# dackey-wav/3d-reconstruction-tool

Measured on AMD Instinct MI355X. Metric: Mpixel-hypotheses/s (PatchMatch sweep), higher is better.
Workload: dtype f32; 1 GPU; BASELINE config 3: 16-view 1920x1080 PatchMatch MVS, 8 iters x (2+8) hypotheses, 7x7 NCC, 4 sources, fast arithmetic; views_per_gpu=16, scene_views=16, width=1920, height=1080, patch=7, iters=8, samples=8, arithmetic=fast, sampling=u8-pairs, tile_rows=18, views_per_launch=4, schedule=auto, exchange=depth + normal + confidence maps once per sweep

## Files before the change

3d-reconstruction-tool_amd/_lib.py:

```python
import ctypes as C
import os

_HERE = os.path.dirname(os.path.abspath(__file__))
LIB_PATH = os.environ.get("AMVS_LIB") or os.path.join(_HERE, "libamvs.so")

AMVS_MAX_SRC = 6
MODES = {"default": 0, "exact": 1, "fast": 2}
SCHEDULES = {"auto": 0, "view-major": 1, "band-major": 2, "split": 3, "paired": 4}
SUPPORTED_PATCH_SIZES = tuple(range(3, 32, 2))
TSDF_MAX_POINTS = 1 << 27

f32p = C.POINTER(C.c_float)
i32p = C.POINTER(C.c_int)


class PmParams(C.Structure):
    _fields_ = [("patch_size", C.c_int32), ("num_iterations", C.c_int32),
                ("num_samples", C.c_int32), ("tile_rows", C.c_int32), ("views_per_launch", C.c_int32),
                ("depth_min", C.c_float), ("depth_max", C.c_float),
                ("log_depth_scale", C.c_float), ("log_depth_min", C.c_float), ("mode", C.c_int32),
                ("schedule", C.c_int32), ("first_iteration", C.c_int32), ("flags", C.c_int32)]


PM_NO_CONFIDENCE = 1
# ... 2 lines not shown
class XpmParams(C.Structure):
    _fields_ = [("patch_size", C.c_int32), ("window_stride", C.c_int32), ("num_refine", C.c_int32),
                ("view_propagation", C.c_int32), ("depth_min", C.c_float), ("depth_max", C.c_float),
                ("log_depth_scale", C.c_float), ("log_depth_min", C.c_float),
                ("consistency_px", C.c_float), ("consistency_rel", C.c_float)]


class Timing(C.Structure):
    _fields_ = [("init_ms", C.c_double), ("sweep_ms", C.c_double), ("confidence_ms", C.c_double),
                ("sweep_launches", C.c_int64), ("pixel_hypotheses", C.c_int64)]


SIGNATURES = {
    "amvs_version": (C.c_char_p, []),
    "amvs_last_error": (C.c_char_p, [C.c_void_p]),
    "amvs_create": (C.c_int, [C.c_int, C.c_int, C.c_int, C.c_int, f32p, f32p, C.POINTER(C.c_void_p)]),
    "amvs_destroy": (C.c_int, [C.c_void_p]),
    "amvs_set_stream": (C.c_int, [C.c_void_p, C.c_void_p]),
    "amvs_sync": (C.c_int, [C.c_void_p]),
    "amvs_set_view": (C.c_int, [C.c_void_p, C.c_int, f32p, f32p, f32p]),
    "amvs_set_view_device": (C.c_int, [C.c_void_p, C.c_int, C.c_void_p, f32p, f32p]),
    "amvs_set_view_bgr8": (C.c_int, [C.c_void_p, C.c_int, C.POINTER(C.c_uint8), C.c_int, C.c_int, f32p, f32p,
                                     C.POINTER(C.c_uint8)]),
    "amvs_patchmatch": (C.c_int, [C.c_void_p, C.c_int, i32p, i32p, C.c_int, C.POINTER(PmParams),
                                  C.c_uint64, f32p, f32p, f32p]),
    "amvs_patchmatch_device": (C.c_int, [C.c_void_p, C.c_int, i32p, i32p, C.c_int,
                                         C.POINTER(PmParams), C.c_uint64,
                                         C.c_void_p, C.c_void_p, C.c_void_p]),
    "amvs_get_timing": (C.c_int, [C.c_void_p, C.POINTER(Timing)]),
    "amvs_sampling_mode": (C.c_int, [C.c_void_p]),
    "amvs_set_sampling": (C.c_int, [C.c_void_p, C.c_int]),
    "amvs_set_mode": (C.c_int, [C.c_void_p, C.c_int]),
    "amvs_get_mode": (C.c_int, [C.c_void_p]),
    "amvs_set_sweep_tuning": (C.c_int, [C.c_void_p, C.c_int, C.c_int]),
    "amvs_set_split_tuning": (C.c_int, [C.c_void_p, C.c_int, C.c_int, C.c_int]),
    "amvs_set_step_tuning": (C.c_int, [C.c_void_p, C.c_int, i32p, i32p]),
    "amvs_set_step_timing": (C.c_int, [C.c_void_p, C.c_int]),
    "amvs_get_step_times": (C.c_int, [C.c_void_p, f32p, C.c_int, i32p]),
    "amvs_last_tile_rows": (C.c_int, [C.c_void_p]),
    "amvs_last_views_per_launch": (C.c_int, [C.c_void_p]),
    "amvs_plane_sweep": (C.c_int, [C.c_void_p, C.c_int, i32p, C.c_int, f32p, C.c_int, C.c_int,
                                   C.c_float, f32p, f32p]),
    "amvs_plane_sweep_device": (C.c_int, [C.c_void_p, C.c_int, i32p, i32p, C.c_int, f32p, C.c_int,
                                          C.c_int, C.c_float, C.c_void_p, C.c_void_p]),
    "amvs_plane_sweep_batch": (C.c_int, [C.c_void_p, C.c_int, i32p, i32p, C.c_int, f32p, C.c_int, C.c_int, C.c_float]),
    "amvs_fetch_sweep_maps": (C.c_int, [C.c_void_p, C.c_int, C.c_int, f32p, f32p]),
# ... 100 lines not shown
```

3d-reconstruction-tool_amd/core/dense_stereo.py:

```python
import threading
import time
from typing import Dict, List, Optional, Tuple

import numpy as np

from .camera import Camera, CameraPose
from .imageprep import prepare_views
from .. import engine as _engine
from .. import parallel as _parallel


def _torch_cuda():
    try:
        import torch
    except Exception:
        return None
    return torch if torch.cuda.is_available() else None


_DRAW_BUF = threading.local()


class DenseStereoReconstructor:
    NUM_NEIGHBORS = 6
# ... 4 lines not shown
                 process_group=None, device_prep: Optional[bool] = None):
        self.camera = camera
        self.scale = scale
        self.num_depths = num_depths
        self.patch_size = patch_size
        self.min_views = min_views
        self.consistency_thresh = consistency_thresh
        self.device_id = _parallel.local_device() if device is None else int(device)
        self.device_filter = device_filter
        self.process_group = process_group
        from . import imageprep as _ip
        self.device_prep = (_ip._cv is None) if device_prep is None else bool(device_prep)
        if mode not in ("exact", "fast"):
            raise ValueError("mode must be 'exact' or 'fast'")
        self.mode = mode
        print(f"Dense stereo using GPU: HIP device {self.device_id} (gfx950 kernels)")
        self.K_scaled = camera.K.copy()
        for r, c in ((0, 0), (1, 1), (0, 2), (1, 2)):
            self.K_scaled[r, c] *= scale
        self._engine = None
        self._engine_key = None
        self._engine_images = None
        self._resident_colors = False
        self._slot = {}

    def reconstruct(self, images: List[dict], poses: Dict[int, CameraPose],
                    max_pairs: int = 30) -> Tuple[np.ndarray, np.ndarray]:
        print("\n" + "=" * 60)
        print("GPU DENSE STEREO")
        print(f"  Scale: {self.scale}x, Depths: {self.num_depths}, Min views: {self.min_views}")
        print("=" * 60)
        t0 = time.time()
        camera_indices = sorted(poses.keys())
        n_cameras = len(camera_indices)
        if n_cameras < 3:
            print("Need at least 3 cameras for multi-view stereo")
            return np.array([]), np.array([])

        print("\nPreparing images...")
        if self.device_prep:
            processed = self._prepare_images_device(images, camera_indices, poses)
        else:
            processed = self._prepare_images(images, camera_indices)

        centers = np.array([poses[idx].center for idx in camera_indices])
        radius = np.percentile(np.linalg.norm(centers - np.median(centers, axis=0), axis=1), 90)
# ... 130 lines not shown

    def _draw_without_replacement(self, total: int, size: int) -> np.ndarray:
        buf = getattr(_DRAW_BUF, "pair", None)
        if buf is None or buf[0].size < total:
            cap = max(int(total), 1 << 20)
            buf = _DRAW_BUF.pair = (np.arange(cap, dtype=np.int64), np.empty(cap, np.int64))
        idx = buf[1][:total]
        np.copyto(idx, buf[0][:total])
        np.random.shuffle(idx)
        return idx[:size]

    def _prepare_images(self, images: List[dict], indices: List[int]) -> Dict:
        return dict(zip(indices, prepare_views([images[idx]["image"] for idx in indices], self.scale)))

    def _prepare_images_device(self, images: List[dict], indices: List[int], poses: Dict[int, CameraPose]) -> Dict:
        h, w = images[indices[0]]["image"].shape[:2]
        H, W = int(h * self.scale), int(w * self.scale)
        eng = self._engine
        if eng is None or not eng.reusable_for(H, W, len(indices), self.K_scaled, self.device_id, self.mode):
            if eng is not None:
                eng.close()
                self._engine = None
            eng = _engine.Engine(H, W, len(indices), self.K_scaled.astype(np.float32), device=self.device_id, mode=self.mode)
        self._slot = {idx: s for s, idx in enumerate(indices)}
        prepared = {}
        for idx in indices:
            img = images[idx]["image"]
            same = (H, W) == tuple(img.shape[:2])
            color = eng.set_view_bgr8(self._slot[idx], img, poses[idx].R, poses[idx].t, want_color=not same)
            prepared[idx] = {"color": img if same else color, "gray": None, "shape": (H, W)}
        self._engine, self._engine_images, self._resident_colors = eng, prepared, True
        self._engine_key = self._make_engine_key(prepared, poses)
        return prepared

    def _make_engine_key(self, processed: Dict, poses: Dict[int, CameraPose]):
        indices = sorted(processed.keys())
        H, W = processed[indices[0]]["shape"]
        pose_print = b"".join(np.asarray(poses[i].R, np.float64).tobytes() + np.asarray(poses[i].t, np.float64).tobytes()
                              for i in indices)
        return (tuple(indices), (int(H), int(W)), pose_print, self.K_scaled.tobytes(), self.device_id)

    def _find_neighbors(self, ref_idx: int, all_indices: List[int],
                        poses: Dict[int, CameraPose], k: int = 6) -> List[int]:
        c_ref = poses[ref_idx].center
        ranked = sorted(((idx, np.linalg.norm(poses[idx].center - c_ref))
                         for idx in all_indices if idx != ref_idx), key=lambda item: item[1])
        return [idx for idx, _ in ranked[:k]]

    def _ensure_engine(self, processed: Dict, poses: Dict[int, CameraPose]):
        indices = sorted(processed.keys())
        H, W = processed[indices[0]]["shape"]
        key = self._make_engine_key(processed, poses)
        if self._engine is not None and self._engine_images is processed and self._engine_key == key:
            return self._engine
# ... 79 lines not shown
```

3d-reconstruction-tool_amd/core/mvs_patchmatch.py:

```python
import time
from dataclasses import dataclass
from typing import Dict, List, Optional, Tuple

import numpy as np

from .camera import Camera, CameraPose
from .imageprep import prepare_view, prepare_views
from .. import engine as _engine
from .. import parallel as _parallel


@dataclass
class DepthNormalMap:
    depth: np.ndarray
    normal: np.ndarray
    confidence: np.ndarray


@dataclass
class _ResidentMaps:
    ref_ids: list
    depth: object
    normal: object
    confidence: object
# ... 34 lines not shown
        self.num_iterations = num_iterations
        self.num_samples = num_samples
        self.min_views = min_views
        self.depth_min = depth_min
        self.depth_max = depth_max
        self.seed = seed
        self.views_per_batch = max(1, int(views_per_batch))
        self.process_group = process_group
        self.device_fusion = device_fusion
        self.device_prep = (not _imageprep_has_cv2()) if device_prep is None else bool(device_prep)
        self.gather_normals = gather_normals
        self.extended = extended
        if mode not in ("exact", "fast"):
            raise ValueError("mode must be 'exact' or 'fast'")
        self.mode = mode
        self.device_id = _parallel.local_device() if device is None else int(device)
        print(f"PatchMatch MVS using GPU: HIP device {self.device_id} (gfx950 kernels)")
        self.K_scaled = camera.K.copy()
        self.K_scaled[:2] *= scale
        self._engine = None
        self._engine_key = None
        self._engine_images = None
        self._resident_colors = False
        self._slot = {}
        self.last_timing = None

    def reconstruct(self, images: List[dict], poses: Dict[int, CameraPose],
                    sparse_points: np.ndarray = None) -> Tuple[np.ndarray, np.ndarray]:
        points, colors, _ = self._reconstruct_maps(images, poses, sparse_points)
        return points, colors

    def reconstruct_mesh(self, images: List[dict], poses: Dict[int, CameraPose], sparse_points: np.ndarray = None, *,
                         voxel_size: Optional[float] = None, bounds=None, trunc_voxels: float = 4.0,
                         max_dim: int = 256) -> Tuple[np.ndarray, np.ndarray, np.ndarray]:
        rank, world = _parallel.rank_world(self.process_group)
        if world > 1:
            raise NotImplementedError("reconstruct_mesh runs on one process: meshing with a process group of "
                                      f"{world} ranks is not implemented (call it without a process group)")
        if trunc_voxels <= 0:
            raise ValueError("trunc_voxels must be positive")
        points, _, maps = self._reconstruct_maps(images, poses, sparse_points)
        empty = (np.zeros((0, 3), np.float32), np.zeros((0, 3), np.int32), np.zeros((0, 3), np.uint8))
        if maps is None or (bounds is None and len(points) == 0):
            return empty
        origin, voxel, dims, trunc = self._mesh_grid(points, bounds, voxel_size, trunc_voxels, max_dim)
        print(f"\nMeshing: {dims[0]} x {dims[1]} x {dims[2]} TSDF grid, voxel {voxel:.4g}, truncation {trunc:.4g}")
# ... 128 lines not shown
                    pooled.extend(z)
            if pooled:
                self.depth_min = max(0.1, np.percentile(pooled, 1))
                self.depth_max = np.percentile(pooled, 99) * 1.5
                return
        spread = np.linalg.norm(centers - np.median(centers, axis=0), axis=1)
        scene_scale = np.percentile(spread, 90)
        self.depth_min = max(0.1, scene_scale * 0.05)
        self.depth_max = scene_scale * 10.0

    def _prepare_images(self, images: List[dict], indices: List[int]) -> Dict:
        prepared = prepare_views([images[idx]["image"] for idx in indices], self.scale)
        return dict(zip(indices, prepared))

    def _prepare_images_device(self, images: List[dict], indices: List[int], poses: Dict[int, CameraPose]) -> Dict:
        h, w = images[indices[0]]["image"].shape[:2]
        H, W = int(h * self.scale), int(w * self.scale)
        eng = self._engine
        if eng is None or not eng.reusable_for(H, W, len(indices), self.K_scaled, self.device_id):
            if eng is not None:
                eng.close()
                self._engine = None
            eng = _engine.Engine(H, W, len(indices), self.K_scaled.astype(np.float32), device=self.device_id)
        self._slot = {idx: s for s, idx in enumerate(indices)}
        prepared = {}
        for idx in indices:
            img = images[idx]["image"]
            if img.shape[:2] != (h, w):
                raise ValueError("all views must share one size")
            same = (H, W) == (h, w)
            color = eng.set_view_bgr8(self._slot[idx], img, poses[idx].R, poses[idx].t, want_color=not same)
            prepared[idx] = {"color": img if same else color, "gray": None, "shape": (H, W)}
        self._engine, self._engine_images, self._resident_colors = eng, prepared, True
        self._engine_key = self._make_engine_key(prepared, poses, indices)
        return prepared

    def _make_engine_key(self, images: Dict, poses: Dict[int, CameraPose], indices: List[int]):
        H, W = images[indices[0]]["shape"]
        pose_print = b"".join(np.asarray(poses[i].R, np.float64).tobytes() + np.asarray(poses[i].t, np.float64).tobytes()
                              for i in indices)
        return (tuple(indices), (int(H), int(W)), pose_print, self.K_scaled.tobytes(), self.device_id)

    def _select_source_views(self, ref_idx: int, all_indices: List[int],
                             poses: Dict[int, CameraPose], k: int = 4) -> List[int]:
        c_ref = poses[ref_idx].center
        z_ref = poses[ref_idx].R[2, :]
        scored = []
        for idx in all_indices:
            if idx == ref_idx:
                continue
            baseline = np.linalg.norm(poses[idx].center - c_ref)
            cosang = np.clip(np.dot(z_ref, poses[idx].R[2, :]), -1, 1)
            angle = np.degrees(np.arccos(cosang))
            score = baseline * (1 - abs(angle - 20) / 60) if 5 < angle < 60 else 0
            scored.append((idx, score))
        scored.sort(key=lambda item: item[1], reverse=True)
# ... 339 lines not shown
```

3d-reconstruction-tool_amd/csrc/amvs_capi.hip:

```cpp
#include "../../include/amvs.h"
#include "amvs_kernels.h"
#include "amvs_buffer.h"

#include <dlfcn.h>
#include <rccl/rccl.h>

#include <array>
#include <cmath>
#include <cstdio>
#include <cstdlib>
#include <cstring>
#include <map>
#include <memory>
#include <string>
#include <vector>

static_assert(AMVS_MAX_SRC == AMVS_KMAX_SRC, "source-count limits out of sync");

#ifdef AMVS_CHECK_INDICES
namespace amvs {
void check_fetch_kernels(unsigned long long out[4], bool reset);
void check_fetch_kernels_fast(unsigned long long out[4], bool reset);
void check_fetch_sweep_fast(unsigned long long out[4], bool reset);
void check_fetch_sweep_exact(unsigned long long out[4], bool reset);
void check_fetch_generic(unsigned long long out[4], bool reset);
void check_fetch_extended(unsigned long long out[4], bool reset);
void check_fetch_fusion(unsigned long long out[4], bool reset);
void check_fetch_knn(unsigned long long out[4], bool reset);
void check_fetch_mesh(unsigned long long out[4], bool reset);
}
#endif

namespace {

std::string g_create_error;

void index_report(uint64_t out[4], bool reset)
{
    out[0] = out[1] = out[2] = out[3] = 0;
#ifdef AMVS_CHECK_INDICES
    (void)hipDeviceSynchronize();
    void (*const fetch[])(unsigned long long[4], bool) = {
        amvs::check_fetch_kernels, amvs::check_fetch_kernels_fast, amvs::check_fetch_sweep_fast, amvs::check_fetch_sweep_exact,
        amvs::check_fetch_generic, amvs::check_fetch_extended, amvs::check_fetch_fusion, amvs::check_fetch_knn,
        amvs::check_fetch_mesh};
    for (auto f : fetch) {
        unsigned long long r[4] = {0, 0, 0, 0};
        f(r, reset);
        if (r[0] && !out[0]) { out[1] = r[1]; out[2] = r[2]; out[3] = r[3]; }
        out[0] += r[0];
    }
#else
    (void)reset;
#endif
}

struct Stats {
    amvs::DeviceBuffer<float> mean, var;
    std::vector<char> done;
};

struct FastStats {
    amvs::DeviceBuffer<float2> maps;
    std::vector<char> done;
};

struct Cloud {
    amvs::DeviceBuffer<double> pts;
    amvs::DeviceBuffer<unsigned char> rgb;
    long long n = 0;
};

}

struct amvs_ctx {
    int device = 0, H = 0, W = 0, n_views = 0, n_cu = 256;
    long long stride = 0;
    float K[9], Kinv[9];
    std::vector<std::array<float, 9>> R;
    std::vector<std::array<float, 3>> t;
    std::vector<char> have;
    amvs::ScratchCache cache;
    amvs::DeviceBuffer<float> d_images;
    amvs::DeviceBuffer<uint16_t> d_pairs;
    long long pstride = 0;
    amvs::DeviceBuffer<unsigned char> d_bgr;
    amvs::DeviceBuffer<unsigned char> d_prep_src;
    amvs::DeviceBuffer<int> d_prep_tab;
    std::vector<char> have_bgr;
    amvs::DeviceBuffer<int> d_flag;
    mutable std::vector<char> exact8;
    mutable bool flags_dirty = false;
    bool force_f32 = false;
    int mode = AMVS_MODE_EXACT;
    int default_band_major = 0;
    int sweep_tile_rows = 0, sweep_chunk = 0;
    int sweep_key8 = 1;
    std::map<int, Stats> stats;
    std::map<int, FastStats> fstats;
    amvs::DeviceBuffer<float> d_depth[2], d_cost, d_normal[2], d_aux;
    amvs::DeviceBuffer<amvs::Job> d_jobs;
    amvs::DeviceBuffer<float> d_planes;
    amvs::DeviceBuffer<unsigned> d_keys;
    amvs::DeviceBuffer<float> d_xcand_d, d_xcand_n;
    amvs::DeviceBuffer<int> d_xsrc;
    amvs::DeviceBuffer<float> d_sweep_depth, d_sweep_conf;
    int n_sweep = 0;
    Cloud cloud;
    std::unique_ptr<amvs::TsdfState, void (*)(amvs::TsdfState *)> tsdf{nullptr, amvs::tsdf_state_free};
    amvs::DeviceBuffer<float> d_samples;
    std::vector<hipStream_t> split_streams;
// ... 647 lines not shown
    c->stream = c->own_stream;
    for (auto &ev : c->ev) HIPCHK(nullptr, hipEventCreate(&ev));
    HIPCHK(nullptr, c->d_images.reserve(c->stride * n_views, c->cache));
    HIPCHK(nullptr, hipMemsetAsync(c->d_images.get(), 0, sizeof(float) * c->stride * n_views, c->stream));
    HIPCHK(nullptr, c->d_pairs.reserve(c->pstride * n_views, c->cache));
    HIPCHK(nullptr, hipMemsetAsync(c->d_pairs.get(), 0, sizeof(uint16_t) * c->pstride * n_views, c->stream));
    HIPCHK(nullptr, c->d_flag.reserve(n_views, c->cache));
    HIPCHK(nullptr, hipMemsetAsync(c->d_flag.get(), 0, sizeof(int) * n_views, c->stream));
    *out = c.release();
    return AMVS_OK;
}

int amvs_destroy(amvs_ctx *c)
{
    if (!c) return AMVS_OK;
    (void)hipSetDevice(c->device);
    if (c->stream) (void)hipStreamSynchronize(c->stream);
    (void)amvs_comm_destroy(c);
    for (auto &st : c->split_streams) (void)hipStreamDestroy(st);
    for (auto &ev : c->split_events) (void)hipEventDestroy(ev);
    for (auto &ev : c->ev) if (ev) (void)hipEventDestroy(ev);
    for (auto &ev : c->ev_groups) (void)hipEventDestroy(ev);
    for (auto &ev : c->ev_steps) (void)hipEventDestroy(ev);
    if (c->own_stream) (void)hipStreamDestroy(c->own_stream);
    delete c;
    return AMVS_OK;
}

int amvs_set_stream(amvs_ctx *c, void *hip_stream)
{
    if (!c) return AMVS_EINVAL;
    c->stream = hip_stream ? (hipStream_t)hip_stream : c->own_stream;
    return AMVS_OK;
}

int amvs_sync(amvs_ctx *c)
{
    if (!c) return AMVS_EINVAL;
    int rc = bind_device(c);
    if (rc) return rc;
    HIPCHK(c, hipStreamSynchronize(c->stream));
    resolve_timing(c);
    return checked(c, AMVS_OK);
}

static int view_uploaded(amvs_ctx *c, int view, const float R[9], const float t[3], bool sync)
// ... 25 lines not shown
    if ((rc = view_uploaded(c, view, R, t, kind == hipMemcpyHostToDevice))) return rc;
    return checked(c, AMVS_OK);
}

static void resize_axis_tables(int n_dst, int n_src, std::vector<int> &ofs, std::vector<short> &w, bool clamp_ofs)
{
    const double scale = 1.0 / ((double)n_dst / (double)n_src);
    ofs.resize(n_dst); w.resize(2 * (size_t)n_dst);
    for (int d = 0; d < n_dst; ++d) {
        float f = (float)((d + 0.5) * scale - 0.5);
        int s = (int)std::floor(f);
        f -= (float)s;
        if (clamp_ofs) {
            if (s < 0) { f = 0.f; s = 0; }
            if (s >= n_src - 1) { f = 0.f; s = n_src - 1; }
        }
        ofs[d] = s;
        const float c0 = 1.f - f, c1 = f;
        w[2 * d] = (short)std::nearbyint(c0 * 2048.f);
        w[2 * d + 1] = (short)std::nearbyint(c1 * 2048.f);
    }
}

int amvs_set_view_bgr8(amvs_ctx *c, int view, const uint8_t *bgr_host, int src_h, int src_w, const float R[9],
                       const float t[3], uint8_t *scaled_bgr_out)
{
    if (c) c->pm_resumable = false;
    if (!c) return AMVS_EINVAL;
    if (view < 0 || view >= c->n_views || !bgr_host || !R || !t || src_h < 1 || src_w < 1)
        return fail(c, AMVS_EINVAL, "bad view argument");
    int rc = bind_device(c);
    if (rc) return rc;
    const size_t n_src = (size_t)src_h * src_w, n_dst = (size_t)c->H * c->W;
    std::vector<int> xofs, yofs;
    std::vector<short> ialpha, ibeta;
    resize_axis_tables(c->W, src_w, xofs, ialpha, true);
    resize_axis_tables(c->H, src_h, yofs, ibeta, false);
    HIPCHK(c, c->d_bgr.reserve(3 * n_dst * (size_t)c->n_views, c->cache));
    unsigned char *d_scaled = c->d_bgr.get() + 3 * n_dst * (size_t)view;
    const size_t tab_ints = (size_t)c->W + c->H, tab_shorts = 2 * ((size_t)c->W + c->H);
    HIPCHK(c, c->d_prep_src.reserve(3 * n_src, c->cache));
    HIPCHK(c, c->d_prep_tab.reserve(tab_ints + tab_shorts / 2, c->cache));
    unsigned char *d_src = c->d_prep_src.get();
    int *d_xofs = c->d_prep_tab.get(), *d_yofs = d_xofs + c->W;
    short *d_ialpha = (short *)(d_xofs + tab_ints), *d_ibeta = d_ialpha + 2 * c->W;
    HIPCHK(c, hipMemcpyAsync(d_src, bgr_host, 3 * n_src, hipMemcpyHostToDevice, c->stream));
    HIPCHK(c, hipMemcpyAsync(d_xofs, xofs.data(), 4 * (size_t)c->W, hipMemcpyHostToDevice, c->stream));
    HIPCHK(c, hipMemcpyAsync(d_yofs, yofs.data(), 4 * (size_t)c->H, hipMemcpyHostToDevice, c->stream));
    HIPCHK(c, hipMemcpyAsync(d_ialpha, ialpha.data(), 4 * (size_t)c->W, hipMemcpyHostToDevice, c->stream));
    HIPCHK(c, hipMemcpyAsync(d_ibeta, ibeta.data(), 4 * (size_t)c->H, hipMemcpyHostToDevice, c->stream));
    HIPCHK(c, amvs::launch_prep_bgr8(d_src, src_h, src_w, c->H, c->W, d_xofs, d_ialpha, d_yofs, d_ibeta, d_scaled,
                                     c->d_images.get() + view * c->stride, c->stream));
    if (scaled_bgr_out) HIPCHK(c, hipMemcpyAsync(scaled_bgr_out, d_scaled, 3 * n_dst, hipMemcpyDeviceToHost, c->stream));
    if ((rc = view_uploaded(c, view, R, t, true))) return rc;
    c->have_bgr[view] = 1;
    return checked(c, AMVS_OK);
}

int amvs_set_view_colors(amvs_ctx *c, int view, const uint8_t *bgr_host)
{
    if (!c) return AMVS_EINVAL;
    if (view < 0 || view >= c->n_views || !bgr_host) return fail(c, AMVS_EINVAL, "bad view argument");
    int rc = bind_device(c);
    if (rc) return rc;
    const size_t n = (size_t)c->H * c->W;
    HIPCHK(c, c->d_bgr.reserve(3 * n * (size_t)c->n_views, c->cache));
    HIPCHK(c, hipMemcpyAsync(c->d_bgr.get() + 3 * n * (size_t)view, bgr_host, 3 * n, hipMemcpyHostToDevice, c->stream));
    HIPCHK(c, hipStreamSynchronize(c->stream));
    c->have_bgr[view] = 1;
    return checked(c, AMVS_OK);
}

int amvs_set_view(amvs_ctx *c, int view, const float *gray_host, const float R[9], const float t[3])
{
    return set_view_common(c, view, gray_host, R, t, hipMemcpyHostToDevice);
}

int amvs_set_view_device(amvs_ctx *c, int view, const void *gray_device, const float R[9], const float t[3])
{
// ... 1038 lines not shown
```

3d-reconstruction-tool_amd/csrc/amvs_prep.hip:

```cpp
#include "amvs_kernels.h"

namespace amvs {

__global__ __launch_bounds__(256) void prep_resize_bgr8_kernel(const unsigned char *__restrict__ src, int sh, int sw,
                                                               int dh, int dw, const int *__restrict__ xofs,
                                                               const short *__restrict__ ialpha,
                                                               const int *__restrict__ yofs,
                                                               const short *__restrict__ ibeta,
                                                               unsigned char *__restrict__ dst)
{
    const long long n = (long long)dh * dw;
    for (long long i = (long long)blockIdx.x * blockDim.x + threadIdx.x; i < n;
         i += (long long)gridDim.x * blockDim.x) {
        const int dy = (int)(i / dw), dx = (int)(i - (long long)dy * dw);
        const int sx0 = xofs[dx], sx1 = sx0 + 1 < sw ? sx0 + 1 : sw - 1;
        const int a0 = ialpha[2 * dx], a1 = ialpha[2 * dx + 1];
        const int b0 = ibeta[2 * dy], b1 = ibeta[2 * dy + 1];
        int sy0 = yofs[dy], sy1 = yofs[dy] + 1;
        sy0 = sy0 < 0 ? 0 : (sy0 > sh - 1 ? sh - 1 : sy0);
        sy1 = sy1 < 0 ? 0 : (sy1 > sh - 1 ? sh - 1 : sy1);
        const unsigned char *r0 = src + (long long)sy0 * sw * 3, *r1 = src + (long long)sy1 * sw * 3;
#pragma unroll
        for (int c = 0; c < 3; ++c) {
            const int D0 = r0[3 * sx0 + c] * a0 + r0[3 * sx1 + c] * a1;
            const int D1 = r1[3 * sx0 + c] * a0 + r1[3 * sx1 + c] * a1;
            dst[3 * i + c] = (unsigned char)((((b0 * (D0 >> 4)) >> 16) + ((b1 * (D1 >> 4)) >> 16) + 2) >> 2);
        }
    }
}

__global__ __launch_bounds__(256) void prep_gray_kernel(const unsigned char *__restrict__ bgr, long long n,
                                                        float *__restrict__ gray)
{
    for (long long i = (long long)blockIdx.x * blockDim.x + threadIdx.x; i < n;
         i += (long long)gridDim.x * blockDim.x) {
        const unsigned v = (bgr[3 * i] * 3735u + bgr[3 * i + 1] * 19235u + bgr[3 * i + 2] * 9798u + 16384u) >> 15;
        gray[i] = (float)v / 255.0f;
    }
}

hipError_t launch_prep_bgr8(const unsigned char *src, int sh, int sw, int dh, int dw, const int *xofs,
                            const short *ialpha, const int *yofs, const short *ibeta, unsigned char *scaled,
                            float *gray, hipStream_t st)
{
    const long long n = (long long)dh * dw;
    const dim3 grid((unsigned)((n + 255) / 256 < 8192 ? (n + 255) / 256 : 8192)), blk(256);
    if (sh == dh && sw == dw) {
        hipError_t e = hipMemcpyAsync(scaled, src, 3 * n, hipMemcpyDeviceToDevice, st);
        if (e != hipSuccess) return e;
    } else {
        hipLaunchKernelGGL(prep_resize_bgr8_kernel, grid, blk, 0, st, src, sh, sw, dh, dw, xofs, ialpha, yofs, ibeta, scaled);
    }
    hipLaunchKernelGGL(prep_gray_kernel, grid, blk, 0, st, scaled, n, gray);
    return hipGetLastError();
}

}
```

3d-reconstruction-tool_amd/engine.py:

```python
import ctypes as C

import numpy as np

from . import _lib
from ._lib import AmvsError, PmParams, Timing, XpmParams, f32p, i32p


def _f32(a, shape=None):
    a = np.ascontiguousarray(a, dtype=np.float32)
    if shape is not None and a.shape != shape:
        raise ValueError(f"expected shape {shape}, got {a.shape}")
    return a


def _p(a):
    return a.ctypes.data_as(f32p)


def _ids(a):
    a = np.ascontiguousarray(a, dtype=np.int32)
    return a, a.ctypes.data_as(i32p)


def make_pm_params(patch_size, num_iterations, num_samples, depth_min, depth_max, tile_rows=0,
                   views_per_launch=0, mode="default", schedule="auto", first_iteration=0, confidence=True):
    log_min = np.log(float(depth_min))
    log_max = np.log(float(depth_max))
    return PmParams(int(patch_size), int(num_iterations), int(num_samples), int(tile_rows),
                    int(views_per_launch), float(depth_min), float(depth_max),
                    float(np.float32(log_max - log_min)), float(np.float32(log_min)), _lib.MODES[mode],
                    _lib.SCHEDULES[schedule], int(first_iteration), 0 if confidence else _lib.PM_NO_CONFIDENCE)


def make_xpm_params(patch_size, depth_min, depth_max, window_stride=2, num_refine=2, view_propagation=True,
                    consistency_px=1.0, consistency_rel=0.01):
    log_min = np.log(float(depth_min))
    log_max = np.log(float(depth_max))
    return XpmParams(int(patch_size), int(window_stride), int(num_refine), int(bool(view_propagation)),
                     float(depth_min), float(depth_max), float(np.float32(log_max - log_min)), float(np.float32(log_min)),
                     float(consistency_px), float(consistency_rel))


class Engine:
    def __init__(self, H, W, n_views, K, K_inv=None, device=0, mode="exact"):
        self._lib = _lib.load()
        self.H, self.W, self.n_views, self.device = int(H), int(W), int(n_views), int(device)
        self.K = _f32(np.asarray(K, np.float32).reshape(3, 3))
        if K_inv is None:
            K_inv = np.linalg.inv(self.K)
        self.K_inv = _f32(np.asarray(K_inv, np.float32).reshape(3, 3))
        h = C.c_void_p()
        rc = self._lib.amvs_create(self.device, self.H, self.W, self.n_views, _p(self.K), _p(self.K_inv),
                                   C.byref(h))
        if rc != 0:
            raise AmvsError(f"amvs_create failed ({rc}): {self._lib.amvs_last_error(None).decode()}")
        self._h = h
        if mode != "exact":
            self.set_mode(mode)

    def reusable_for(self, H, W, n_views, K, device, mode="exact"):
        return (self._h is not None and (self.H, self.W, self.n_views, self.device) == (int(H), int(W), int(n_views), int(device))
                and np.array_equal(self.K, np.asarray(K, np.float32).reshape(3, 3)) and self.mode() == mode)

# ... 78 lines not shown
    def sync(self):
        self._chk(self._lib.amvs_sync(self._h))

    def set_stream(self, stream_ptr):
        self._chk(self._lib.amvs_set_stream(self._h, C.c_void_p(stream_ptr or 0)))

    def set_view(self, view, gray, R, t):
        gray = _f32(gray, (self.H, self.W))
        R = _f32(np.asarray(R, np.float64).astype(np.float32).reshape(3, 3))
        t = _f32(np.asarray(t, np.float64).astype(np.float32).reshape(3))
        self._chk(self._lib.amvs_set_view(self._h, int(view), _p(gray), _p(R), _p(t)))

    def set_view_bgr8(self, view, image_bgr_u8, R, t, want_color=True):
        img = np.ascontiguousarray(image_bgr_u8, dtype=np.uint8)
        if img.ndim != 3 or img.shape[2] != 3:
            raise ValueError("expected an (h, w, 3) uint8 BGR image")
        R = _f32(np.asarray(R, np.float64).astype(np.float32).reshape(3, 3))
        t = _f32(np.asarray(t, np.float64).astype(np.float32).reshape(3))
        out = np.empty((self.H, self.W, 3), np.uint8) if want_color else None
        self._chk(self._lib.amvs_set_view_bgr8(
            self._h, int(view), img.ctypes.data_as(C.POINTER(C.c_uint8)), img.shape[0], img.shape[1], _p(R), _p(t),
            out.ctypes.data_as(C.POINTER(C.c_uint8)) if want_color else None))
        return out

    def set_view_colors(self, view, image_bgr_u8):
        img = np.ascontiguousarray(image_bgr_u8, dtype=np.uint8)
        if img.shape != (self.H, self.W, 3):
            raise ValueError(f"expected a ({self.H}, {self.W}, 3) uint8 BGR image")
        self._chk(self._lib.amvs_set_view_colors(self._h, int(view), img.ctypes.data_as(C.POINTER(C.c_uint8))))

    def set_view_device(self, view, gray_ptr, R, t):
        R = _f32(np.asarray(R, np.float64).astype(np.float32).reshape(3, 3))
        t = _f32(np.asarray(t, np.float64).astype(np.float32).reshape(3))
        self._chk(self._lib.amvs_set_view_device(self._h, int(view), C.c_void_p(gray_ptr), _p(R), _p(t)))

    def patchmatch(self, ref_ids, src_ids, params, seed):
        ref, refp = _ids(ref_ids)
        src, srcp = _ids(src_ids)
        n = ref.shape[0]
        src = src.reshape(n, -1)
        depth = np.empty((n, self.H, self.W), np.float32)
        normal = np.empty((n, self.H, self.W, 3), np.float32)
        conf = np.empty((n, self.H, self.W), np.float32)
        self._chk(self._lib.amvs_patchmatch(self._h, n, refp, srcp, src.shape[1], C.byref(params),
                                            int(seed), _p(depth), _p(normal), _p(conf)))
        return depth, normal, conf
# ... 371 lines not shown
```

include/amvs.h:

```cpp
#ifndef AMVS_H
#define AMVS_H

#include <stdint.h>

#ifdef __cplusplus
extern "C" {
#endif

#define AMVS_MAX_SRC 6

#define AMVS_OK            0
#define AMVS_EINVAL       -1
#define AMVS_EHIP         -2
#define AMVS_EINDEX       -4
#define AMVS_EUNSUPPORTED -3

typedef struct amvs_ctx amvs_ctx;

#define AMVS_MODE_DEFAULT 0
#define AMVS_MODE_EXACT   1
#define AMVS_MODE_FAST    2

typedef struct {
    int32_t patch_size;
// ... 21 lines not shown
    double  init_ms;
    double  sweep_ms;
    double  confidence_ms;
    int64_t sweep_launches;
    int64_t pixel_hypotheses;
} amvs_timing;

const char *amvs_version(void);
const char *amvs_last_error(const amvs_ctx *ctx);

int amvs_create(int device_id, int H, int W, int n_views,
                const float K[9], const float K_inv[9], amvs_ctx **out);
int amvs_destroy(amvs_ctx *ctx);
int amvs_set_stream(amvs_ctx *ctx, void *hip_stream);
int amvs_sync(amvs_ctx *ctx);

int amvs_set_view(amvs_ctx *ctx, int view, const float *gray_host,
                  const float R[9], const float t[3]);
int amvs_set_view_device(amvs_ctx *ctx, int view, const void *gray_device,
                         const float R[9], const float t[3]);

int amvs_set_view_bgr8(amvs_ctx *ctx, int view, const uint8_t *bgr_host, int src_h, int src_w,
                       const float R[9], const float t[3], uint8_t *scaled_bgr_out);

int amvs_patchmatch(amvs_ctx *ctx, int n_ref, const int *ref_ids, const int *src_ids,
                    int n_src, const amvs_pm_params *p, uint64_t seed,
                    float *depth_out, float *normal_out, float *conf_out);
int amvs_patchmatch_device(amvs_ctx *ctx, int n_ref, const int *ref_ids, const int *src_ids,
                           int n_src, const amvs_pm_params *p, uint64_t seed,
                           void *depth_dev, void *normal_dev, void *conf_dev);
int amvs_get_timing(const amvs_ctx *ctx, amvs_timing *out);
int amvs_sampling_mode(const amvs_ctx *ctx);
int amvs_set_sampling(amvs_ctx *ctx, int force_f32);
int amvs_set_mode(amvs_ctx *ctx, int mode);
int amvs_get_mode(const amvs_ctx *ctx);
int amvs_set_sweep_tuning(amvs_ctx *ctx, int tile_rows, int planes_per_wave);
int amvs_set_step_tuning(amvs_ctx *ctx, int n_iterations, const int32_t *tile_rows, const int32_t *wgs_per_cu);
int amvs_set_step_timing(amvs_ctx *ctx, int enable);
int amvs_get_step_times(amvs_ctx *ctx, float *ms_out, int capacity, int *n_out);
int amvs_set_split_tuning(amvs_ctx *ctx, int groups, int sample_rows, int sample_lds_bytes);
int amvs_last_tile_rows(const amvs_ctx *ctx);
int amvs_last_views_per_launch(const amvs_ctx *ctx);

int amvs_plane_sweep(amvs_ctx *ctx, int ref, const int *nbr_ids, int n_nbr,
                     const float *depths, int D, int patch_size, float thresh,
                     float *depth_out, float *conf_out);
// ... 107 lines not shown
```

Before: 44440 Mpx-hyp/s.

## Batch BGR view uploads with double-buffered copy stream and row-compacted transfers

Adds a batched set_views_bgr8 path that uploads all views through a separate copy stream with two staging buffers, so the host-to-device copy of one view can overlap the resize kernel of the previous one. When downscaling only touches a regular subset of source rows, it uploads just those rows using a strided 2D copy and resizes with a new compact-row kernel. It also caches the resize tables on the device and reuses host color buffers from a pool. All of this sits in image preparation, not in the PatchMatch sweep, so the sweep throughput metric is unlikely to be affected.

```diff
diff --git a/3d-reconstruction-tool_amd/_lib.py b/3d-reconstruction-tool_amd/_lib.py
--- a/3d-reconstruction-tool_amd/_lib.py
+++ b/3d-reconstruction-tool_amd/_lib.py
@@ -48,6 +48,10 @@
     "amvs_set_view_device": (C.c_int, [C.c_void_p, C.c_int, C.c_void_p, f32p, f32p]),
     "amvs_set_view_bgr8": (C.c_int, [C.c_void_p, C.c_int, C.POINTER(C.c_uint8), C.c_int, C.c_int, f32p, f32p,
                                      C.POINTER(C.c_uint8)]),
+    "amvs_set_views_bgr8": (C.c_int, [C.c_void_p, C.c_int, i32p, C.POINTER(C.c_void_p), C.c_int, C.c_int, f32p, f32p,
+                                      C.POINTER(C.c_void_p)]),
+    "amvs_set_upload_rows": (C.c_int, [C.c_void_p, C.c_int]),
+    "amvs_upload_plan": (C.c_int, [C.c_void_p, C.c_int, C.c_int, i32p]),
     "amvs_patchmatch": (C.c_int, [C.c_void_p, C.c_int, i32p, i32p, C.c_int, C.POINTER(PmParams),
                                   C.c_uint64, f32p, f32p, f32p]),
     "amvs_patchmatch_device": (C.c_int, [C.c_void_p, C.c_int, i32p, i32p, C.c_int,
diff --git a/3d-reconstruction-tool_amd/core/dense_stereo.py b/3d-reconstruction-tool_amd/core/dense_stereo.py
--- a/3d-reconstruction-tool_amd/core/dense_stereo.py
+++ b/3d-reconstruction-tool_amd/core/dense_stereo.py
@@ -50,6 +50,7 @@
         self._engine_key = None
         self._engine_images = None
         self._resident_colors = False
+        self._color_pool = _engine.HostBufferPool()
         self._slot = {}
 
     def reconstruct(self, images: List[dict], poses: Dict[int, CameraPose],
@@ -226,14 +227,17 @@
                 eng.close()
                 self._engine = None
             eng = _engine.Engine(H, W, len(indices), self.K_scaled.astype(np.float32), device=self.device_id, mode=self.mode)
+        self._engine_key = self._engine_images = None
+        self._engine = eng
         self._slot = {idx: s for s, idx in enumerate(indices)}
-        prepared = {}
-        for idx in indices:
-            img = images[idx]["image"]
-            same = (H, W) == tuple(img.shape[:2])
-            color = eng.set_view_bgr8(self._slot[idx], img, poses[idx].R, poses[idx].t, want_color=not same)
-            prepared[idx] = {"color": img if same else color, "gray": None, "shape": (H, W)}
-        self._engine, self._engine_images, self._resident_colors = eng, prepared, True
+        imgs = [images[idx]["image"] for idx in indices]
+        same = (H, W) == (h, w)
+        out = None if same else self._color_pool.take((len(indices), H, W, 3))
+        eng.set_views_bgr8([self._slot[idx] for idx in indices], imgs, [poses[idx].R for idx in indices],
+                           [poses[idx].t for idx in indices], want_color=not same, color_out=out)
+        prepared = {idx: {"color": imgs[k] if same else out[k], "gray": None, "shape": (H, W)}
+                    for k, idx in enumerate(indices)}
+        self._engine_images, self._resident_colors = prepared, True
         self._engine_key = self._make_engine_key(prepared, poses)
         return prepared
 
diff --git a/3d-reconstruction-tool_amd/core/mvs_patchmatch.py b/3d-reconstruction-tool_amd/core/mvs_patchmatch.py
--- a/3d-reconstruction-tool_amd/core/mvs_patchmatch.py
+++ b/3d-reconstruction-tool_amd/core/mvs_patchmatch.py
@@ -80,6 +80,7 @@
         self._engine_key = None
         self._engine_images = None
         self._resident_colors = False
+        self._color_pool = _engine.HostBufferPool()
         self._slot = {}
         self.last_timing = None
 
@@ -254,16 +255,20 @@
                 eng.close()
                 self._engine = None
             eng = _engine.Engine(H, W, len(indices), self.K_scaled.astype(np.float32), device=self.device_id)
+        self._engine_key = self._engine_images = None
+        self._engine = eng
         self._slot = {idx: s for s, idx in enumerate(indices)}
-        prepared = {}
-        for idx in indices:
-            img = images[idx]["image"]
+        imgs = [images[idx]["image"] for idx in indices]
+        for img in imgs:
             if img.shape[:2] != (h, w):
                 raise ValueError("all views must share one size")
-            same = (H, W) == (h, w)
-            color = eng.set_view_bgr8(self._slot[idx], img, poses[idx].R, poses[idx].t, want_color=not same)
-            prepared[idx] = {"color": img if same else color, "gray": None, "shape": (H, W)}
-        self._engine, self._engine_images, self._resident_colors = eng, prepared, True
+        same = (H, W) == (h, w)
+        out = None if same else self._color_pool.take((len(indices), H, W, 3))
+        eng.set_views_bgr8([self._slot[idx] for idx in indices], imgs, [poses[idx].R for idx in indices],
+                           [poses[idx].t for idx in indices], want_color=not same, color_out=out)
+        prepared = {idx: {"color": imgs[k] if same else out[k], "gray": None, "shape": (H, W)}
+                    for k, idx in enumerate(indices)}
+        self._engine_images, self._resident_colors = prepared, True
         self._engine_key = self._make_engine_key(prepared, poses, indices)
         return prepared
 
diff --git a/3d-reconstruction-tool_amd/csrc/amvs_capi.hip b/3d-reconstruction-tool_amd/csrc/amvs_capi.hip
--- a/3d-reconstruction-tool_amd/csrc/amvs_capi.hip
+++ b/3d-reconstruction-tool_amd/csrc/amvs_capi.hip
@@ -1,6 +1,7 @@
 #include "../../include/amvs.h"
 #include "amvs_kernels.h"
 #include "amvs_buffer.h"
+#include "amvs_prep.h"
 
 #include <dlfcn.h>
 #include <rccl/rccl.h>
@@ -28,6 +29,7 @@
 void check_fetch_fusion(unsigned long long out[4], bool reset);
 void check_fetch_knn(unsigned long long out[4], bool reset);
 void check_fetch_mesh(unsigned long long out[4], bool reset);
+void check_fetch_prep(unsigned long long out[4], bool reset);
 }
 #endif
 
@@ -43,7 +45,7 @@
     void (*const fetch[])(unsigned long long[4], bool) = {
         amvs::check_fetch_kernels, amvs::check_fetch_kernels_fast, amvs::check_fetch_sweep_fast, amvs::check_fetch_sweep_exact,
         amvs::check_fetch_generic, amvs::check_fetch_extended, amvs::check_fetch_fusion, amvs::check_fetch_knn,
-        amvs::check_fetch_mesh};
+        amvs::check_fetch_mesh, amvs::check_fetch_prep};
     for (auto f : fetch) {
         unsigned long long r[4] = {0, 0, 0, 0};
         f(r, reset);
@@ -69,6 +71,15 @@
     amvs::DeviceBuffer<double> pts;
     amvs::DeviceBuffer<unsigned char> rgb;
     long long n = 0;
+};
+
+struct PrepPlan {
+    int src_h = 0, src_w = 0;
+    bool compact = false;
+    int first_row = 0, run_rows = 0, stride_rows = 0, n_runs = 0, n_rows = 0;
+    std::vector<int> tab_i;
+    std::vector<short> tab_s;
+    bool on_device = false;
 };
 
 }
@@ -87,6 +98,10 @@
     amvs::DeviceBuffer<unsigned char> d_bgr;
     amvs::DeviceBuffer<unsigned char> d_prep_src;
     amvs::DeviceBuffer<int> d_prep_tab;
+    PrepPlan prep_plan;
+    bool upload_rows = true;
+    hipStream_t copy_stream = nullptr;
+    hipEvent_t ev_staged[2] = {nullptr, nullptr}, ev_consumed[2] = {nullptr, nullptr};
     std::vector<char> have_bgr;
     amvs::DeviceBuffer<int> d_flag;
     mutable std::vector<char> exact8;
@@ -780,6 +795,9 @@
     for (auto &ev : c->ev) if (ev) (void)hipEventDestroy(ev);
     for (auto &ev : c->ev_groups) (void)hipEventDestroy(ev);
     for (auto &ev : c->ev_steps) (void)hipEventDestroy(ev);
+    if (c->copy_stream) { (void)hipStreamSynchronize(c->copy_stream); (void)hipStreamDestroy(c->copy_stream); }
+    for (auto &ev : c->ev_staged) if (ev) (void)hipEventDestroy(ev);
+    for (auto &ev : c->ev_consumed) if (ev) (void)hipEventDestroy(ev);
     if (c->own_stream) (void)hipStreamDestroy(c->own_stream);
     delete c;
     return AMVS_OK;
@@ -851,39 +869,167 @@
     }
 }
 
+static void build_prep_plan(amvs_ctx *c, int src_h, int src_w)
+{
+    PrepPlan &p = c->prep_plan;
+    if (p.src_h == src_h && p.src_w == src_w) return;
+    p = PrepPlan();
+    p.src_h = src_h; p.src_w = src_w;
+    const int H = c->H, W = c->W;
+    std::vector<int> xofs, yofs;
+    std::vector<short> ialpha, ibeta;
+    resize_axis_tables(W, src_w, xofs, ialpha, true);
+    resize_axis_tables(H, src_h, yofs, ibeta, false);
+    auto clamp_row = [src_h](int r) { return r < 0 ? 0 : (r > src_h - 1 ? src_h - 1 : r); };
+    std::vector<char> used(src_h, 0);
+    for (int dy = 0; dy < H; ++dy) used[clamp_row(yofs[dy])] = used[clamp_row(yofs[dy] + 1)] = 1;
+    std::vector<std::pair<int, int>> runs;
+    int kept = 0;
+    for (int r = 0; r < src_h; ++r) {
+        if (!used[r]) continue;
+        ++kept;
+        if (!runs.empty() && runs.back().first + runs.back().second == r) ++runs.back().second;
+        else runs.emplace_back(r, 1);
+    }
+    bool uniform = runs.size() >= 2 && 3ll * kept <= 2ll * src_h && !(src_h == H && src_w == W);
+    const int first = runs[0].first, len = runs[0].second, stride = runs.size() >= 2 ? runs[1].first - first : 0;
+    for (size_t i = 0; uniform && i < runs.size(); ++i) {
+        if (runs[i].first != first + (int)i * stride) uniform = false;
+        if (runs[i].second != len) uniform = false;
+    }
+    std::vector<int> row0(H, 0), row1(H, 0);
+    if (uniform) {
+        p.compact = true;
+        p.first_row = first; p.run_rows = len; p.stride_rows = stride;
+        p.n_runs = (int)runs.size();
+        p.n_rows = p.n_runs * len;
+        auto compact_row = [&](int r) { return (r - first) / stride * len + (r - first) % stride; };
+        for (int dy = 0; dy < H; ++dy) {
+            row0[dy] = compact_row(clamp_row(yofs[dy]));
+            row1[dy] = compact_row(clamp_row(yofs[dy] + 1));
+        }
+    }
+    p.tab_i.reserve((size_t)W + 3 * (size_t)H);
+    p.tab_i.insert(p.tab_i.end(), xofs.begin(), xofs.end());
+    p.tab_i.insert(p.tab_i.end(), yofs.begin(), yofs.end());
+    p.tab_i.insert(p.tab_i.end(), row0.begin(), row0.end());
+    p.tab_i.insert(p.tab_i.end(), row1.begin(), row1.end());
+    p.tab_s = ialpha;
+    p.tab_s.insert(p.tab_s.end(), ibeta.begin(), ibeta.end());
+}
+
+static int set_views_bgr8_queue(amvs_ctx *c, int n, const int *view_ids, const uint8_t *const *bgr_hosts, int src_h,
+                                int src_w, const float *R, const float *t, uint8_t *const *scaled_bgr_outs)
+{
+    const size_t n_dst = (size_t)c->H * c->W, row_bytes = 3 * (size_t)src_w;
+    build_prep_plan(c, src_h, src_w);
+    PrepPlan &p = c->prep_plan;
+    const bool compact = p.compact && c->upload_rows;
+    const size_t stage_bytes = (row_bytes * (size_t)(compact ? p.n_rows : src_h) + 255) & ~size_t(255);
+    HIPCHK(c, c->d_bgr.reserve(3 * n_dst * (size_t)c->n_views, c->cache));
+    HIPCHK(c, c->d_prep_src.reserve(stage_bytes * (n > 1 ? 2 : 1), c->cache));
+    const size_t tab_ints = p.tab_i.size(), tab_shorts = p.tab_s.size();
+    if (c->d_prep_tab.capacity() < tab_ints + tab_shorts / 2) p.on_device = false;
+    HIPCHK(c, c->d_prep_tab.reserve(tab_ints + tab_shorts / 2, c->cache));
+    int *d_xofs = c->d_prep_tab.get(), *d_yofs = d_xofs + c->W, *d_row0 = d_yofs + c->H, *d_row1 = d_row0 + c->H;
+    short *d_ialpha = (short *)(d_xofs + tab_ints), *d_ibeta = d_ialpha + 2 * c->W;
+    if (!p.on_device) {
+        HIPCHK(c, hipMemcpyAsync(d_xofs, p.tab_i.data(), 4 * tab_ints, hipMemcpyHostToDevice, c->stream));
+        HIPCHK(c, hipMemcpyAsync(d_ialpha, p.tab_s.data(), 2 * tab_shorts, hipMemcpyHostToDevice, c->stream));
+        p.on_device = true;
+    }
+    if (!c->copy_stream) {
+        HIPCHK(c, hipStreamCreateWithFlags(&c->copy_stream, hipStreamNonBlocking));
+        for (auto &ev : c->ev_staged) HIPCHK(c, hipEventCreateWithFlags(&ev, hipEventDisableTiming));
+        for (auto &ev : c->ev_consumed) HIPCHK(c, hipEventCreateWithFlags(&ev, hipEventDisableTiming));
+    }
+    auto upload = [&](int k) -> int {
+        const int b = k & 1;
+        unsigned char *d_src = c->d_prep_src.get() + stage_bytes * b;
+        if (k >= 2) HIPCHK(c, hipStreamWaitEvent(c->copy_stream, c->ev_consumed[b], 0));
+        if (compact) {
+            const size_t run_bytes = row_bytes * p.run_rows;
+            HIPCHK(c, hipMemcpy2DAsync(d_src, run_bytes, bgr_hosts[k] + row_bytes * p.first_row, row_bytes * p.stride_rows,
+                                       run_bytes, p.n_runs, hipMemcpyHostToDevice, c->copy_stream));
+        } else {
+            HIPCHK(c, hipMemcpyAsync(d_src, bgr_hosts[k], row_bytes * src_h, hipMemcpyHostToDevice, c->copy_stream));
+        }
+        HIPCHK(c, hipEventRecord(c->ev_staged[b], c->copy_stream));
+        return AMVS_OK;
+    };
+    int rc = upload(0);
+    if (rc) return rc;
+    for (int k = 0; k < n; ++k) {
+        const int b = k & 1, view = view_ids[k];
+        unsigned char *d_src = c->d_prep_src.get() + stage_bytes * b;
+        unsigned char *d_scaled = c->d_bgr.get() + 3 * n_dst * (size_t)view;
+        float *d_gray = c->d_images.get() + view * c->stride;
+        HIPCHK(c, hipStreamWaitEvent(c->stream, c->ev_staged[b], 0));
+        if (compact)
+            HIPCHK(c, amvs::launch_prep_bgr8_rows(d_src, p.n_rows, src_w, c->H, c->W, d_xofs, d_ialpha, d_row0, d_row1,
+                                                  d_ibeta, d_scaled, d_gray, c->stream));
+        else
+            HIPCHK(c, amvs::launch_prep_bgr8(d_src, src_h, src_w, c->H, c->W, d_xofs, d_ialpha, d_yofs, d_ibeta, d_scaled,
+                                             d_gray, c->stream));
+        HIPCHK(c, hipEventRecord(c->ev_consumed[b], c->stream));
+        if ((rc = view_uploaded(c, view, R + 9 * (size_t)k, t + 3 * (size_t)k, false))) return rc;
+        c->have_bgr[view] = 1;
+        if (k + 1 < n && (rc = upload(k + 1))) return rc;
+    }
+    for (int k = 0; scaled_bgr_outs && k < n;) {
+        int m = 1;
+        if (!scaled_bgr_outs[k]) { ++k; continue; }
+        while (k + m < n && view_ids[k + m] == view_ids[k] + m && scaled_bgr_outs[k + m] == scaled_bgr_outs[k] + 3 * n_dst * m) ++m;
+        HIPCHK(c, hipMemcpyAsync(scaled_bgr_outs[k], c->d_bgr.get() + 3 * n_dst * (size_t)view_ids[k], 3 * n_dst * m,
+                                 hipMemcpyDeviceToHost, c->stream));
+        k += m;
+    }
+    HIPCHK(c, hipStreamSynchronize(c->stream));
+    return AMVS_OK;
+}
+
+int amvs_set_views_bgr8(amvs_ctx *c, int n, const int *view_ids, const uint8_t *const *bgr_hosts, int src_h, int src_w,
+                        const float *R, const float *t, uint8_t *const *scaled_bgr_outs)
+{
+    if (c) c->pm_resumable = false;
+    if (!c) return AMVS_EINVAL;
+    if (n < 1 || !view_ids || !bgr_hosts || !R || !t || src_h < 1 || src_w < 1) return fail(c, AMVS_EINVAL, "bad view argument");
+    std::vector<char> listed(c->n_views, 0);
+    for (int k = 0; k < n; ++k) {
+        if (view_ids[k] < 0 || view_ids[k] >= c->n_views || !bgr_hosts[k]) return fail(c, AMVS_EINVAL, "bad view argument");
+        if (listed[view_ids[k]]++) return fail(c, AMVS_EINVAL, "bad view argument: view " + std::to_string(view_ids[k]) + " listed twice");
+    }
+    int rc = bind_device(c);
+    if (rc) return rc;
+    rc = set_views_bgr8_queue(c, n, view_ids, bgr_hosts, src_h, src_w, R, t, scaled_bgr_outs);
+    if (rc) {
+        if (c->copy_stream) (void)hipStreamSynchronize(c->copy_stream);
+        (void)hipStreamSynchronize(c->stream);
+        return rc;
+    }
+    return checked(c, AMVS_OK);
+}
+
 int amvs_set_view_bgr8(amvs_ctx *c, int view, const uint8_t *bgr_host, int src_h, int src_w, const float R[9],
                        const float t[3], uint8_t *scaled_bgr_out)
 {
-    if (c) c->pm_resumable = false;
-    if (!c) return AMVS_EINVAL;
-    if (view < 0 || view >= c->n_views || !bgr_host || !R || !t || src_h < 1 || src_w < 1)
-        return fail(c, AMVS_EINVAL, "bad view argument");
-    int rc = bind_device(c);
-    if (rc) return rc;
-    const size_t n_src = (size_t)src_h * src_w, n_dst = (size_t)c->H * c->W;
-    std::vector<int> xofs, yofs;
-    std::vector<short> ialpha, ibeta;
-    resize_axis_tables(c->W, src_w, xofs, ialpha, true);
-    resize_axis_tables(c->H, src_h, yofs, ibeta, false);
-    HIPCHK(c, c->d_bgr.reserve(3 * n_dst * (size_t)c->n_views, c->cache));
-    unsigned char *d_scaled = c->d_bgr.get() + 3 * n_dst * (size_t)view;
-    const size_t tab_ints = (size_t)c->W + c->H, tab_shorts = 2 * ((size_t)c->W + c->H);
-    HIPCHK(c, c->d_prep_src.reserve(3 * n_src, c->cache));
-    HIPCHK(c, c->d_prep_tab.reserve(tab_ints + tab_shorts / 2, c->cache));
-    unsigned char *d_src = c->d_prep_src.get();
-    int *d_xofs = c->d_prep_tab.get(), *d_yofs = d_xofs + c->W;
-    short *d_ialpha = (short *)(d_xofs + tab_ints), *d_ibeta = d_ialpha + 2 * c->W;
-    HIPCHK(c, hipMemcpyAsync(d_src, bgr_host, 3 * n_src, hipMemcpyHostToDevice, c->stream));
-    HIPCHK(c, hipMemcpyAsync(d_xofs, xofs.data(), 4 * (size_t)c->W, hipMemcpyHostToDevice, c->stream));
-    HIPCHK(c, hipMemcpyAsync(d_yofs, yofs.data(), 4 * (size_t)c->H, hipMemcpyHostToDevice, c->stream));
-    HIPCHK(c, hipMemcpyAsync(d_ialpha, ialpha.data(), 4 * (size_t)c->W, hipMemcpyHostToDevice, c->stream));
-    HIPCHK(c, hipMemcpyAsync(d_ibeta, ibeta.data(), 4 * (size_t)c->H, hipMemcpyHostToDevice, c->stream));
-    HIPCHK(c, amvs::launch_prep_bgr8(d_src, src_h, src_w, c->H, c->W, d_xofs, d_ialpha, d_yofs, d_ibeta, d_scaled,
-                                     c->d_images.get() + view * c->stride, c->stream));
-    if (scaled_bgr_out) HIPCHK(c, hipMemcpyAsync(scaled_bgr_out, d_scaled, 3 * n_dst, hipMemcpyDeviceToHost, c->stream));
-    if ((rc = view_uploaded(c, view, R, t, true))) return rc;
-    c->have_bgr[view] = 1;
-    return checked(c, AMVS_OK);
+    return amvs_set_views_bgr8(c, 1, &view, &bgr_host, src_h, src_w, R, t, &scaled_bgr_out);
+}
+
+int amvs_upload_plan(amvs_ctx *c, int src_h, int src_w, int *rows_uploaded)
+{
+    if (!c) return AMVS_EINVAL;
+    if (src_h < 1 || src_w < 1 || !rows_uploaded) return fail(c, AMVS_EINVAL, "bad source size");
+    build_prep_plan(c, src_h, src_w);
+    *rows_uploaded = c->prep_plan.compact && c->upload_rows ? c->prep_plan.n_rows : src_h;
+    return AMVS_OK;
+}
+
+int amvs_set_upload_rows(amvs_ctx *c, int enable)
+{
+    if (!c) return AMVS_EINVAL;
+    c->upload_rows = enable != 0;
+    return AMVS_OK;
 }
 
 int amvs_set_view_colors(amvs_ctx *c, int view, const uint8_t *bgr_host)
diff --git a/3d-reconstruction-tool_amd/csrc/amvs_prep.h b/3d-reconstruction-tool_amd/csrc/amvs_prep.h
--- /dev/null
+++ b/3d-reconstruction-tool_amd/csrc/amvs_prep.h
@@ -0,0 +1,10 @@
+#pragma once
+#include <hip/hip_runtime.h>
+
+namespace amvs {
+
+hipError_t launch_prep_bgr8_rows(const unsigned char *src, int n_rows, int sw, int dh, int dw, const int *xofs,
+                                 const short *ialpha, const int *row0, const int *row1, const short *ibeta,
+                                 unsigned char *scaled, float *gray, hipStream_t st);
+
+}
diff --git a/3d-reconstruction-tool_amd/csrc/amvs_prep.hip b/3d-reconstruction-tool_amd/csrc/amvs_prep.hip
--- a/3d-reconstruction-tool_amd/csrc/amvs_prep.hip
+++ b/3d-reconstruction-tool_amd/csrc/amvs_prep.hip
@@ -1,4 +1,7 @@
+#define AMVS_TU_ID 10
+#include "amvs_check.h"
 #include "amvs_kernels.h"
+#include "amvs_prep.h"
 
 namespace amvs {
 
@@ -20,6 +23,32 @@
         sy0 = sy0 < 0 ? 0 : (sy0 > sh - 1 ? sh - 1 : sy0);
         sy1 = sy1 < 0 ? 0 : (sy1 > sh - 1 ? sh - 1 : sy1);
         const unsigned char *r0 = src + (long long)sy0 * sw * 3, *r1 = src + (long long)sy1 * sw * 3;
+#pragma unroll
+        for (int c = 0; c < 3; ++c) {
+            const int D0 = r0[3 * sx0 + c] * a0 + r0[3 * sx1 + c] * a1;
+            const int D1 = r1[3 * sx0 + c] * a0 + r1[3 * sx1 + c] * a1;
+            dst[3 * i + c] = (unsigned char)((((b0 * (D0 >> 4)) >> 16) + ((b1 * (D1 >> 4)) >> 16) + 2) >> 2);
+        }
+    }
+}
+
+__global__ __launch_bounds__(256) void prep_resize_bgr8_rows_kernel(const unsigned char *__restrict__ src, int n_rows,
+                                                                    int sw, int dh, int dw, const int *__restrict__ xofs,
+                                                                    const short *__restrict__ ialpha,
+                                                                    const int *__restrict__ row0,
+                                                                    const int *__restrict__ row1,
+                                                                    const short *__restrict__ ibeta,
+                                                                    unsigned char *__restrict__ dst)
+{
+    const long long n = (long long)dh * dw;
+    for (long long i = (long long)blockIdx.x * blockDim.x + threadIdx.x; i < n;
+         i += (long long)gridDim.x * blockDim.x) {
+        const int dy = (int)(i / dw), dx = (int)(i - (long long)dy * dw);
+        const int sx0 = AMVS_IDX(xofs[dx], sw), sx1 = sx0 + 1 < sw ? sx0 + 1 : sw - 1;
+        const int a0 = ialpha[2 * dx], a1 = ialpha[2 * dx + 1];
+        const int b0 = ibeta[2 * dy], b1 = ibeta[2 * dy + 1];
+        const int cy0 = AMVS_IDX(row0[dy], n_rows), cy1 = AMVS_IDX(row1[dy], n_rows);
+        const unsigned char *r0 = src + (long long)cy0 * sw * 3, *r1 = src + (long long)cy1 * sw * 3;
 #pragma unroll
         for (int c = 0; c < 3; ++c) {
             const int D0 = r0[3 * sx0 + c] * a0 + r0[3 * sx1 + c] * a1;
@@ -55,4 +84,18 @@
     return hipGetLastError();
 }
 
+hipError_t launch_prep_bgr8_rows(const unsigned char *src, int n_rows, int sw, int dh, int dw, const int *xofs,
+                                 const short *ialpha, const int *row0, const int *row1, const short *ibeta,
+                                 unsigned char *scaled, float *gray, hipStream_t st)
+{
+    const long long n = (long long)dh * dw;
+    const dim3 grid((unsigned)((n + 255) / 256 < 8192 ? (n + 255) / 256 : 8192)), blk(256);
+    hipLaunchKernelGGL(prep_resize_bgr8_rows_kernel, grid, blk, 0, st, src, n_rows, sw, dh, dw, xofs, ialpha, row0, row1,
+                       ibeta, scaled);
+    hipLaunchKernelGGL(prep_gray_kernel, grid, blk, 0, st, scaled, n, gray);
+    return hipGetLastError();
 }
+
+}
+
+AMVS_CHECK_TU(prep)
diff --git a/3d-reconstruction-tool_amd/engine.py b/3d-reconstruction-tool_amd/engine.py
--- a/3d-reconstruction-tool_amd/engine.py
+++ b/3d-reconstruction-tool_amd/engine.py
@@ -1,4 +1,5 @@
 import ctypes as C
+import sys
 
 import numpy as np
 
@@ -39,6 +40,22 @@
     return XpmParams(int(patch_size), int(window_stride), int(num_refine), int(bool(view_propagation)),
                      float(depth_min), float(depth_max), float(np.float32(log_max - log_min)), float(np.float32(log_min)),
                      float(consistency_px), float(consistency_rel))
+
+
+class HostBufferPool:
+
+    def __init__(self, depth=3):
+        self._depth, self._bufs = int(depth), []
+
+    def take(self, shape):
+        shape = tuple(int(x) for x in shape)
+        for buf in self._bufs:
+            if buf.shape == shape and sys.getrefcount(buf) <= 3:
+                return buf
+        buf = np.empty(shape, np.uint8)
+        buf.fill(0)
+        self._bufs = [b for b in self._bufs if b.shape == shape][-(self._depth - 1):] + [buf]
+        return buf
 
 
 class Engine:
@@ -163,6 +180,36 @@
             self._h, int(view), img.ctypes.data_as(C.POINTER(C.c_uint8)), img.shape[0], img.shape[1], _p(R), _p(t),
             out.ctypes.data_as(C.POINTER(C.c_uint8)) if want_color else None))
         return out
+
+    def set_views_bgr8(self, views, images_bgr_u8, Rs, ts, want_color=True, color_out=None):
+        views = np.ascontiguousarray(views, dtype=np.int32).reshape(-1)
+        n = views.shape[0]
+        if n < 1 or not (len(images_bgr_u8) == len(Rs) == len(ts) == n):
+            raise ValueError("expected one image, R and t per view")
+        imgs = [np.ascontiguousarray(im, dtype=np.uint8) for im in images_bgr_u8]
+        h, w = imgs[0].shape[:2]
+        for im in imgs:
+            if im.ndim != 3 or im.shape != (h, w, 3):
+                raise ValueError("expected (h, w, 3) uint8 BGR images of one size")
+        R = _f32(np.stack([np.asarray(r, np.float64).astype(np.float32).reshape(9) for r in Rs]))
+        t = _f32(np.stack([np.asarray(x, np.float64).astype(np.float32).reshape(3) for x in ts]))
+        src = (C.c_void_p * n)(*[im.ctypes.data for im in imgs])
+        out = outs = None
+        if want_color:
+            out = color_out if color_out is not None else np.empty((n, self.H, self.W, 3), np.uint8)
+            if out.shape != (n, self.H, self.W, 3) or out.dtype != np.uint8 or not out.flags.c_contiguous:
+                raise ValueError(f"color_out must be a contiguous ({n}, {self.H}, {self.W}, 3) uint8 array")
+            outs = (C.c_void_p * n)(*[out[k].ctypes.data for k in range(n)])
+        self._chk(self._lib.amvs_set_views_bgr8(self._h, n, views.ctypes.data_as(i32p), src, h, w, _p(R), _p(t), outs))
+        return out
+
+    def set_upload_rows(self, enable=True):
+        self._chk(self._lib.amvs_set_upload_rows(self._h, int(bool(enable))))
+
+    def upload_plan(self, src_h, src_w):
+        rows = C.c_int(0)
+        self._chk(self._lib.amvs_upload_plan(self._h, int(src_h), int(src_w), C.byref(rows)))
+        return rows.value
 
     def set_view_colors(self, view, image_bgr_u8):
         img = np.ascontiguousarray(image_bgr_u8, dtype=np.uint8)
diff --git a/include/amvs.h b/include/amvs.h
--- a/include/amvs.h
+++ b/include/amvs.h
@@ -67,6 +67,10 @@
 
 int amvs_set_view_bgr8(amvs_ctx *ctx, int view, const uint8_t *bgr_host, int src_h, int src_w,
                        const float R[9], const float t[3], uint8_t *scaled_bgr_out);
+int amvs_set_views_bgr8(amvs_ctx *ctx, int n, const int *view_ids, const uint8_t *const *bgr_hosts, int src_h,
+                        int src_w, const float *R, const float *t, uint8_t *const *scaled_bgr_outs);
+int amvs_set_upload_rows(amvs_ctx *ctx, int enable);
+int amvs_upload_plan(amvs_ctx *ctx, int src_h, int src_w, int *rows_uploaded);
 
 int amvs_patchmatch(amvs_ctx *ctx, int n_ref, const int *ref_ids, const int *src_ids,
                     int n_src, const amvs_pm_params *p, uint64_t seed,
```

After: 44420 Mpx-hyp/s, median of 3. No clear change (-0.1%).
